# AIoT-MLSys-Lab/Mercury

Measured on AMD Instinct MI355X. Metric: images/sec (whole node) + sampler overhead %, ResNet-18 CIFAR-10 DP 1/2/4/8 GPU, higher is better.
Workload: dtype bf16; 1 GPU; model=resnet18, dataset=cifar10-shape (32x32x3, 10 classes), global_batch=32, per_gpu_batch=32, presample_pool=320, optimizer=adam, parallelism=dp1, sampler=importance (loss + 0.5*EMA), with replacement

## Files before the change

csrc/bindings.cpp:

```cpp
#include <pybind11/pybind11.h>
#include <pybind11/stl.h>

#include <stdexcept>
#include <string>
#include <vector>

#include "kernels.h"

int igemm_read_stamps(unsigned long long* host, int n);
int conv_bwd_pair_sc_launch(const bf16* dyA, const bf16* wtA, const ConvGeom& gA_in,
                            const EpiParams& eA_in, int bm, int bn, int splits, const bf16* xA,
                            const WgradGeom& wgA_in, float* dwA, int wbm, int wbn, int wsplits,
                            const bf16* dyB, const bf16* wtB, const ConvGeom& gtB,
                            const EpiParams& eB_in, int HB, int WB, int NB, const bf16* xB,
                            const WgradGeom& wgB_in, float* dwB, int wsplitsB, hipStream_t st);
int igemm_dual_launch(const bf16* srcA, const bf16* wtA, const ConvGeom& gA, const EpiParams& eA,
                      int splitsA, const bf16* srcB, const bf16* wtB, const ConvGeom& gB,
                      const EpiParams& eB, int splitsB, int bm, int bn, hipStream_t st);
int hconv_read_stamps(unsigned long long* host, int n);
void hconv_configure(int grid, int waves, int wm8);
std::string comm_unique_id();
uintptr_t comm_init(const std::string& id_bytes, int rank, int nranks);
void comm_destroy(uintptr_t c);
void comm_allreduce(uintptr_t c, uintptr_t buf, long long count, int dtype, int avg, uintptr_t st);
void comm_allgather(uintptr_t c, uintptr_t send, uintptr_t recv, long long count, int dtype,
                    uintptr_t st);
void comm_broadcast(uintptr_t c, uintptr_t buf, long long count, int dtype, int root, uintptr_t st);
void comm_ring_allreduce(uintptr_t c, uintptr_t buf, long long count, uintptr_t work, int avg,
                         uintptr_t st);
void add_f32(float* dst, const float* src, long long n, hipStream_t s);
void xgmi_pack(const float* src, void* xbuf, long long n, int bf, hipStream_t st);
void xgmi_reduce_scatter(const void* const* peers, int W, int rank, long long n, int bf,
                         float scale, hipStream_t st);
void xgmi_all_gather(const void* const* peers, int W, long long n, int bf, float* dst,
                     hipStream_t st);
int xgmi_max_ranks();
void xgmi_barrier(const void* const* flag_areas, int W, int rank, unsigned* epoch,
                  double timeout_s, int* err, hipStream_t st);
int xgmi_flag_bytes();
std::string xgmi_ipc_handle(uintptr_t ptr);
uintptr_t xgmi_ipc_open(const std::string& handle);
uintptr_t xgmi_malloc(long long bytes);
// ... 57 lines not shown
                       int bn, int H, int W, int N, uintptr_t st, uintptr_t bw_out, uintptr_t bw_y,
                       uintptr_t bw_stats, uintptr_t bw_y2, uintptr_t bw_stats2, uintptr_t bw_sums,
                       float bw_inv_count, float bw_eps, int bw_act) {
    ConvGeom g{SH, SW, SC, H, W, R, Sk, stride, pad, R * Sk * SC / 8, Ncols, N * H * W};
    EpiParams e{P<bf16>(dx), ldo, nullptr, nullptr, 0, N * H * W, accumulate, nullptr,
                P<const bf16>(bw_out), P<const bf16>(bw_y), P<const float>(bw_stats),
                P<const bf16>(bw_y2), P<const float>(bw_stats2), P<float>(bw_sums), bw_inv_count,
                bw_eps, bw_act};
    const int ok = dgrad_s2_launch(P<const bf16>(dy), P<const bf16>(wt), g, e, bm, bn, H, W, N,
                                   S(st));
    if (ok) check_launch("dgrad_s2");
    return ok;
  });
  m.def("conv_bwd_pair_s2", [](uintptr_t dy, uintptr_t wt, uintptr_t dx, int ldo, int accumulate,
                               int SH, int SW, int SC, int R, int Sk, int stride, int pad,
                               int Ncols, int bm, int bn, int H, int W, int N, uintptr_t bw_out,
                               uintptr_t bw_y, uintptr_t bw_stats, uintptr_t bw_y2,
                               uintptr_t bw_stats2, uintptr_t bw_sums, float bw_inv_count,
                               float bw_eps, int bw_act, uintptr_t x, uintptr_t dw, int C, int Pp,
                               int Q, int K, int Creal, int wbm, int wbn, int wsplits,
                               uintptr_t wslab, uintptr_t st) {
    ConvGeom g{SH, SW, SC, H, W, R, Sk, stride, pad, R * Sk * SC / 8, Ncols, N * H * W};
    EpiParams e{P<bf16>(dx), ldo, nullptr, nullptr, 0, N * H * W, accumulate, nullptr,
                P<const bf16>(bw_out), P<const bf16>(bw_y), P<const float>(bw_stats),
                P<const bf16>(bw_y2), P<const float>(bw_stats2), P<float>(bw_sums), bw_inv_count,
                bw_eps, bw_act};
    WgradGeom wg{N, H, W, C, Pp, Q, K, R, Sk, stride, pad, Creal, nullptr, P<float>(wslab)};
    const int ok = conv_bwd_pair_s2_launch(P<const bf16>(dy), P<const bf16>(wt), g, e, bm, bn, H,
                                           W, N, P<const bf16>(x), wg, P<float>(dw), wbm, wbn,
                                           wsplits, S(st));
    if (ok) check_launch("conv_bwd_pair_s2");
    return ok;
  });
  m.attr("SUMS_R") = SUMS_R;
  m.def("pgemm", [](uintptr_t a, uintptr_t b, uintptr_t out, uintptr_t stats, int M, int N, int K,
                    int ldo, int stats_ld, int group_rows, long long a_bytes, long long b_bytes,
                    long long out_bytes, int H, int W, int Pp, int Q, int stride, int bn, int grid,
                    uintptr_t st, int p_mode, uintptr_t p_stats, uintptr_t p_rmean,
                    uintptr_t p_rvar, uintptr_t p_gamma, uintptr_t p_beta, float p_inv_count,
                    float p_eps, int p_act, int p_group_rows, int p_G, uintptr_t p_coef,
                    uintptr_t p_res, uintptr_t p_keep, long long p_res_bytes,
                    long long p_keep_bytes, long long p_coef_bytes) {
    const long long lim = 0xFFFFFF00LL;
    if (a_bytes >= lim || b_bytes >= lim || out_bytes >= lim || p_res_bytes >= lim ||
        p_keep_bytes >= lim || p_coef_bytes >= lim)
      throw std::invalid_argument("pgemm: tensors must be < 4 GB (32-bit buffer offsets)");
    PgemmArgs g{P<const bf16>(a), P<const bf16>(b), P<bf16>(out), P<float>(stats), M, N, K, ldo,
                stats_ld, group_rows, (unsigned)a_bytes, (unsigned)b_bytes, (unsigned)out_bytes,
                H, W, Pp, Q, stride};
    PgemmPro pr{p_mode, P<const float>(p_stats), P<const float>(p_rmean), P<const float>(p_rvar),
                P<const float>(p_gamma), P<const float>(p_beta), p_inv_count, p_eps, p_act,
                p_group_rows, p_G, P<float>(p_coef), P<const bf16>(p_res), P<bf16>(p_keep),
                (unsigned)p_res_bytes, (unsigned)p_keep_bytes, (unsigned)p_coef_bytes};
    const int ok = bn == 0 ? pwconv_launch(g, S(st), &pr) : pgemm_launch(g, bn, grid, S(st), &pr);
    check_launch(bn == 0 ? "pwconv" : "pgemm");
    return ok;
  });
  m.def("igemm_pro", [](uintptr_t src, uintptr_t wt, uintptr_t out, int ldo, uintptr_t bias,
                        uintptr_t stats, int stats_ld, int group_rows, uintptr_t slab, int SH,
                        int SW, int SC, int RP, int RQ, int R, int Sk, int stride, int pad, int Kc,
                        int Ncols, int M, int bm, int bn, int splits, uintptr_t st,
                        uintptr_t p_stats, uintptr_t p_rmean, uintptr_t p_rvar, uintptr_t p_gamma,
                        uintptr_t p_beta, uintptr_t p_keep, int p_group_rows, float p_inv_count,
                        float p_eps, int p_act, int p_keep_tap, uintptr_t p_res) {
    ConvGeom g{SH, SW, SC, RP, RQ, R, Sk, stride, pad, Kc, Ncols, M};
    EpiParams e{P<bf16>(out), ldo, P<const float>(bias), P<float>(stats), stats_ld, group_rows, 0,
// ... 595 lines not shown
```

csrc/igemm.hip:

```cpp

#include <stdexcept>
#include <string>

#include "conv_epi.h"
#include "wgrad_body.h"

namespace {


__device__ __attribute__((aligned(16))) bf16 g_zero_page[64];

MA_DEV int swz(int row, int chunk) { return chunk ^ (row & 7); }

template <int BM, int BN>
constexpr int nt_occ() { return BM * BN >= 256 * 128 ? 1 : 2; }


template <bool TRANS>
MA_DEV void row_init(const ConvGeom& g, int m, int& off, int& h, int& w) {
  const int pq = g.RP * g.RQ;
  const int mm = m < g.M ? m : 0;
  const int n = udiv24(mm, pq, 1.f / (float)pq), rem = mm - n * pq;
  const int p = udiv24(rem, g.RQ, 1.f / (float)g.RQ), q = rem - p * g.RQ;
  off = m < g.M ? n * g.SH * g.SW : -1;
// ... 336 lines not shown
    unsigned long long lap[4] = {0, 0, 0, 0};
    unsigned long long tl = __builtin_amdgcn_s_memtime();
#endif
    int buf = 0;
    for (int kt = kt0; kt < kt1; ++kt) {
      const bool more = kt + 1 < kt1;
      if (more) load_stage(kt + 1, ra, rb);
      MA_LAP(0, tl);
      const bf16* a = sA + buf * Smem<BM, BN>::STAGE;
      mma_stage<BM, BN>(a, a + BM * BK, acc, lane, wm, wn);
      MA_LAP(1, tl);
      if (more) store_stage(buf ^ 1, ra, rb);
      MA_LAP(2, tl);
      __syncthreads();
      MA_LAP(3, tl);
      buf ^= 1;
    }
#ifdef MERCURY_STAMPS
    if (threadIdx.x == 0) {
      const int b_ = blockIdx.x + blockIdx.y * gridDim.x;
      if (b_ < 8192)
        for (int q = 0; q < 4; ++q) g_stamps[b_][4 + q] = lap[q];
    }
#endif
  } else if constexpr (EARLY) {
    pf.init(e, g.M, g.Ncols, m0, n0);
    if (pf_tail) epi_prefetch(pf, e, m0, n0, g.Ncols);
  }
  MA_STAMP(2);
  finish<BM, BN, 2, BWT, EARLY>(acc, smem, e, g.M, g.Ncols, m0, n0, bx, by, gx, gy, &pf);
  MA_STAMP(3);
}


template <int BM, int BN>
constexpr int PAIR_PF() { return BM * BN <= 64 * 128 ? 2 : 1; }

template <int BM, int BN, bool TRANS, int PF = 1>
__global__ __launch_bounds__(NT, (nt_occ<BM, BN>())) void igemm_nt_kernel(const bf16* __restrict__ src,
                                                          const bf16* __restrict__ wt,
                                                          ConvGeom g, EpiParams e,
                                                          int ktiles_per_split) {
  __shared__ __attribute__((aligned(16))) char smem[Smem<BM, BN>::bytes(2)];
  const ProParams none{};
  const int bx = gridDim.y == 1 ? xcd_tile(blockIdx.x, gridDim.x) : blockIdx.x;
  igemm_nt_body<BM, BN, TRANS, false, PF>(src, wt, g, e, ktiles_per_split, smem, bx, blockIdx.y,
                                          gridDim.x, gridDim.y, none);
}

template <int BM, int BN>
__global__ __launch_bounds__(NT, (nt_occ<BM, BN>())) void igemm_pro_kernel(const bf16* __restrict__ src,
                                                           const bf16* __restrict__ wt,
                                                           ConvGeom g, EpiParams e,
                                                           int ktiles_per_split, ProParams pro) {
  __shared__ __attribute__((aligned(16))) char smem[Smem<BM, BN>::bytes(2)];
  const int bx = gridDim.y == 1 ? xcd_tile(blockIdx.x, gridDim.x) : blockIdx.x;
  igemm_nt_body<BM, BN, false, true>(src, wt, g, e, ktiles_per_split, smem, bx,
                                     blockIdx.y, gridDim.x, gridDim.y, pro);
}

template <int BM, int BN, bool TRANS>
void launch_main(const bf16* src, const bf16* wt, const ConvGeom& g, const EpiParams& e, int per,
                 dim3 grid, hipStream_t st) {
  if constexpr (PAIR_PF<BM, BN>() == 2) {
#ifndef MERCURY_FWD_PF1
    if (grid.x * grid.y <= 512) {
      hipLaunchKernelGGL((igemm_nt_kernel<BM, BN, TRANS, 2>), grid, dim3(NT), 0, st, src, wt, g, e,
                         per);
      return;
    }
#endif
  }
  hipLaunchKernelGGL((igemm_nt_kernel<BM, BN, TRANS>), grid, dim3(NT), 0, st, src, wt, g, e, per);
}

inline void ig_grid(const ConvGeom& g, int BM, int BN, int splits, int& gx, int& per, int& gy) {
  const int mtiles = (g.M + BM - 1) / BM, ntiles = (g.Ncols + BN - 1) / BN;
  const int ktiles = (g.Kc + 7) / 8;
  splits = splits < 1 ? 1 : (splits > ktiles ? ktiles : splits);
  per = (ktiles + splits - 1) / splits;
  gy = (ktiles + per - 1) / per;
  gx = mtiles * ntiles;
  if (gx > SEM_INTS) gy = 1, per = ktiles;
}

template <int BM, int BN, bool TRANS>
void launch_cfg(const bf16* src, const bf16* wt, const ConvGeom& g, EpiParams e, int splits,
                hipStream_t st, const ProParams* pro) {
  int gx, per, gy;
  ig_grid(g, BM, BN, splits, gx, per, gy);
  if (gy == 1) e.slab = nullptr;
  if (pro != nullptr && !TRANS) {
    hipLaunchKernelGGL((igemm_pro_kernel<BM, BN>), dim3(gx, gy), dim3(NT), 0, st, src, wt, g, e,
                       per, *pro);
    return;
  }
  launch_main<BM, BN, TRANS>(src, wt, g, e, per, dim3(gx, gy), st);
}

struct IgProb {
  const bf16* src;
  const bf16* wt;
  ConvGeom g;
  EpiParams e;
  int per, gx, gy;
};

template <int BM, int BN, int PF>
__global__ __launch_bounds__(NT, (nt_occ<BM, BN>())) void igemm_dual_kernel(IgProb A, IgProb B) {
  __shared__ __attribute__((aligned(16))) char smem[Smem<BM, BN>::bytes(2)];
  const ProParams none{};
  int b = blockIdx.x;
  const bool first = b < A.gx * A.gy;
  if (!first) b -= A.gx * A.gy;
  const IgProb& p = first ? A : B;
  const int bx0 = b % p.gx, by = b / p.gx;
  const int bx = p.gy == 1 ? xcd_tile(bx0, p.gx) : bx0;
  igemm_nt_body<BM, BN, false, false, PF>(p.src, p.wt, p.g, p.e, p.per, smem, bx, by, p.gx, p.gy,
                                          none);
}

template <int BM, int BN>
// ... 30 lines not shown
  const int c = (b >= sg.pre[1]) + (b >= sg.pre[2]) + (b >= sg.pre[3]);
  EpiParams ec = e;
  ec.rm_hc = sg.hc[c];
  ec.rm_wc = sg.wc[c];
  ec.rm_h = sg.H;
  ec.rm_w = sg.W;
  ec.rm_ph = c >> 1;
  ec.rm_pw = c & 1;
  const ProParams none{};
  const int bx = b - sg.pre[c];
  igemm_nt_body<BM, BN, false, false, PF, true>(dy, wt, sg.g[c], ec, 1 << 20, smem, bx, 0,
                                                sg.pre[c + 1] - sg.pre[c], 1, none);
}

template <int BM, int BN>
void s2_cfg(const bf16* dy, const bf16* wt, const S2Geom& sg, const EpiParams& e, hipStream_t st) {
  const int grid = sg.pre[4];
  if (grid == 0) return;
  if constexpr (PAIR_PF<BM, BN>() == 2) {
    if (grid <= 512) {
      hipLaunchKernelGGL((dgrad_s2_kernel<BM, BN, 2>), dim3(grid), dim3(NT), 0, st, dy, wt, sg, e);
      return;
    }
  }
  hipLaunchKernelGGL((dgrad_s2_kernel<BM, BN, 1>), dim3(grid), dim3(NT), 0, st, dy, wt, sg, e);
}

template <int DBM, int DBN, int WBM, int WBN>
__global__ __launch_bounds__(NT, 2) void bwd_pair_kernel(const bf16* __restrict__ dy,
                                                          const bf16* __restrict__ wt, ConvGeom g,
                                                          EpiParams e, int dper, int dgx, int dgy,
                                                          const bf16* __restrict__ x,
                                                          WgradGeom wg, float* __restrict__ dw,
                                                          int wper, int wgx, int wgy) {
  constexpr int DB = Smem<DBM, DBN>::bytes(2), WB = wgb::WgSmem<WBM, WBN>::BYTES;
  __shared__ __attribute__((aligned(16))) char smem[DB > WB ? DB : WB];
  const int nw = wgx * wgy;
  const int b = blockIdx.x;
  if (b < nw) {
    wgb::wgrad_body<WBM, WBN>(dy, x, wg, dw, wper, (bf16*)smem, b % wgx, b / wgx, wgy);
  } else {
    const int d = b - nw;
    const ProParams none{};
    igemm_nt_body<DBM, DBN, true, false, PAIR_PF<DBM, DBN>()>(dy, wt, g, e, dper, smem, d % dgx,
                                                               d / dgx, dgx, dgy, none);
  }
}

template <int DBM, int DBN, int WBM, int WBN>
__global__ __launch_bounds__(NT, 2) void bwd_pair_s2_kernel(const bf16* __restrict__ dy,
                                                             const bf16* __restrict__ wt,
                                                             S2Geom sg, EpiParams e,
                                                             const bf16* __restrict__ x,
                                                             WgradGeom wg, float* __restrict__ dw,
                                                             int wper, int wgx, int wgy) {
  constexpr int DB = Smem<DBM, DBN>::bytes(2), WB = wgb::WgSmem<WBM, WBN>::BYTES;
  __shared__ __attribute__((aligned(16))) char smem[DB > WB ? DB : WB];
  const int nw = wgx * wgy;
  const int b = blockIdx.x;
  if (b < nw) {
    wgb::wgrad_body<WBM, WBN>(dy, x, wg, dw, wper, (bf16*)smem, b % wgx, b / wgx, wgy);
    return;
  }
  const int d = b - nw;
  const int c = (d >= sg.pre[1]) + (d >= sg.pre[2]) + (d >= sg.pre[3]);
  EpiParams ec = e;
  ec.rm_hc = sg.hc[c];
  ec.rm_wc = sg.wc[c];
  ec.rm_h = sg.H;
  ec.rm_w = sg.W;
  ec.rm_ph = c >> 1;
  ec.rm_pw = c & 1;
  const ProParams none{};
  igemm_nt_body<DBM, DBN, false, false, PAIR_PF<DBM, DBN>(), true>(
      dy, wt, sg.g[c], ec, 1 << 20, smem, d - sg.pre[c], 0, sg.pre[c + 1] - sg.pre[c], 1, none);
}

struct PairProb {
  const bf16* dy;
  const bf16* wt;
  ConvGeom g;
  EpiParams e;
  int dper, dgx, dgy;
  const bf16* x;
  WgradGeom wg;
  float* dw;
  int wper, wgx, wgy;
};
struct S2PairProb {
  const bf16* dy;
  const bf16* wt;
  S2Geom sg;
  EpiParams e;
  const bf16* x;
  WgradGeom wg;
  float* dw;
  int wper, wgx, wgy;
};

template <int DBM, int DBN, int WBM, int WBN>
__global__ __launch_bounds__(NT, 2) void bwd_pair_sc_kernel(PairProb A, S2PairProb B) {
  constexpr int DB = Smem<DBM, DBN>::bytes(2), WB = wgb::WgSmem<WBM, WBN>::BYTES;
  constexpr int SB = Smem<64, 64>::bytes(2), SWB = wgb::WgSmem<64, 64>::BYTES;
  constexpr int M1 = DB > WB ? DB : WB, M2 = SB > SWB ? SB : SWB;
  __shared__ __attribute__((aligned(16))) char smem[M1 > M2 ? M1 : M2];
  const ProParams none{};
  int b = blockIdx.x;
  const int nwA = A.wgx * A.wgy, nA = nwA + A.dgx * A.dgy;
  if (b < nA) {
    if (b < nwA) {
      wgb::wgrad_body<WBM, WBN>(A.dy, A.x, A.wg, A.dw, A.wper, (bf16*)smem, b % A.wgx, b / A.wgx,
                                A.wgy);
    } else {
      const int d = b - nwA;
      igemm_nt_body<DBM, DBN, true, false, PAIR_PF<DBM, DBN>()>(A.dy, A.wt, A.g, A.e, A.dper, smem,
                                                                 d % A.dgx, d / A.dgx, A.dgx,
                                                                 A.dgy, none);
    }
    return;
  }
  b -= nA;
  const int nwB = B.wgx * B.wgy;
  if (b < nwB) {
    wgb::wgrad_body<64, 64>(B.dy, B.x, B.wg, B.dw, B.wper, (bf16*)smem, b % B.wgx, b / B.wgx, B.wgy);
    return;
  }
  const int d = b - nwB;
  const int c = (d >= B.sg.pre[1]) + (d >= B.sg.pre[2]) + (d >= B.sg.pre[3]);
  EpiParams ec = B.e;
  ec.rm_hc = B.sg.hc[c];
  ec.rm_wc = B.sg.wc[c];
  ec.rm_h = B.sg.H;
  ec.rm_w = B.sg.W;
  ec.rm_ph = c >> 1;
  ec.rm_pw = c & 1;
  igemm_nt_body<64, 64, false, false, PAIR_PF<64, 64>(), true>(
      B.dy, B.wt, B.sg.g[c], ec, 1 << 20, smem, d - B.sg.pre[c], 0, B.sg.pre[c + 1] - B.sg.pre[c],
      1, none);
}

template <int DBM, int DBN, int WBM, int WBN>
void pair_cfg(const bf16* dy, const bf16* wt, const ConvGeom& g, EpiParams e, int splits,
              const bf16* x, WgradGeom wg, float* dw, int wsplits, hipStream_t st) {
  int dgx, dper, dgy, wgx, wper, wgy;
  ig_grid(g, DBM, DBN, splits, dgx, dper, dgy);
  if (dgy == 1) e.slab = nullptr;
  wgb::wg_grid(wg, WBM, WBN, wsplits, wgx, wper, wgy);
  if (wgx > wgb::WG_SEM_INTS) wg.slab = nullptr;
  hipLaunchKernelGGL((bwd_pair_kernel<DBM, DBN, WBM, WBN>), dim3(dgx * dgy + wgx * wgy), dim3(NT),
                     0, st, dy, wt, g, e, dper, dgx, dgy, x, wg, dw, wper, wgx, wgy);
}

}

int igemm_read_stamps(unsigned long long* host, int n) {
#ifdef MERCURY_STAMPS
  return hipMemcpyFromSymbol(host, HIP_SYMBOL(g_stamps), sizeof(unsigned long long) * 12 * n) ==
         hipSuccess;
#else
  (void)host;
  (void)n;
  return 0;
#endif
}


size_t igemm_slab_bytes(const ConvGeom& g, int bm, int bn, int splits) {
  const size_t mtiles = (g.M + bm - 1) / bm, ntiles = (g.Ncols + bn - 1) / bn;
  return SEM_INTS * 4 + (size_t)splits * mtiles * ntiles * bm * bn * 4;
}

const bf16* conv_zero_page();
static const bf16* zero_page() { return conv_zero_page(); }

const bf16* conv_zero_page() {
  static const bf16* zp = nullptr;
  if (!zp) {
    void* p = nullptr;
    (void)hipGetSymbolAddress(&p, HIP_SYMBOL(g_zero_page));
    zp = (const bf16*)p;
  }
  return zp;
}

void igemm_ranges(ConvGeom& g, long long images, const char* who) {
// ... 147 lines not shown
    wgb::wg_grid(wg, WBM_, WBN_, wsplits, wgx, wper, wgy);                                 \
    if (wgx > wgb::WG_SEM_INTS) wg.slab = nullptr;                                         \
    hipLaunchKernelGGL((bwd_pair_s2_kernel<DBM_, DBN_, WBM_, WBN_>),                        \
                       dim3(sg.pre[4] + wgx * wgy), dim3(NT), 0, st, dy, wt, sg, e, x, wg, dw, \
                       wper, wgx, wgy);                                                    \
    return 1;                                                                              \
  }
  MA_W(64, 64, 64, 64)
  MA_W(64, 64, 128, 128)
  MA_W(64, 64, 64, 128)
  MA_W(64, 64, 128, 64)
#undef MA_W
  return 0;
}

int conv_bwd_pair_sc_launch(const bf16* dyA, const bf16* wtA, const ConvGeom& gA_in,
                            const EpiParams& eA_in, int bm, int bn, int splits, const bf16* xA,
                            const WgradGeom& wgA_in, float* dwA, int wbm, int wbn,
                            int wsplits, const bf16* dyB, const bf16* wtB, const ConvGeom& gtB,
                            const EpiParams& eB_in, int HB, int WB, int NB, const bf16* xB,
                            const WgradGeom& wgB_in, float* dwB, int wsplitsB,
                            hipStream_t st) {
  PairProb A;
  A.dy = dyA;
  A.wt = wtA;
  A.g = gA_in;
  A.g.zero = zero_page();
  igemm_ranges(A.g, geom_images(A.g), "conv_bwd_pair_sc");
  A.e = eA_in;
  A.x = xA;
  A.wg = wgA_in;
  A.wg.zero = A.g.zero;
  A.dw = dwA;
  ig_grid(A.g, bm, bn, splits, A.dgx, A.dper, A.dgy);
  if (A.dgy == 1) A.e.slab = nullptr;
  wgb::wg_grid(A.wg, wbm, wbn, wsplits, A.wgx, A.wper, A.wgy);
  if (A.wgx > wgb::WG_SEM_INTS) A.wg.slab = nullptr;
  S2PairProb B;
  if (!s2_geom(gtB, 64, 64, HB, WB, NB, eB_in.ldo, B.sg)) return 0;
  B.dy = dyB;
  B.wt = wtB;
  B.e = eB_in;
  B.e.slab = nullptr;
  B.x = xB;
  B.wg = wgB_in;
  B.wg.zero = A.g.zero;
  B.dw = dwB;
  wgb::wg_grid(B.wg, 64, 64, wsplitsB, B.wgx, B.wper, B.wgy);
  if (B.wgx > wgb::WG_SEM_INTS) B.wg.slab = nullptr;
  if (A.wg.slab != nullptr && A.wg.slab == B.wg.slab) return 0;
  const int grid = A.wgx * A.wgy + A.dgx * A.dgy + B.wgx * B.wgy + B.sg.pre[4];
#define MA_SC(DBM_, DBN_, WBM_, WBN_)                                                       \
  if (bm == DBM_ && bn == DBN_ && wbm == WBM_ && wbn == WBN_) {                             \
    hipLaunchKernelGGL((bwd_pair_sc_kernel<DBM_, DBN_, WBM_, WBN_>), dim3(grid), dim3(NT), 0, st, \
                       A, B);                                                                \
    return 1;                                                                                \
  }
  MA_SC(64, 64, 64, 64)
  MA_SC(64, 64, 128, 128)
#undef MA_SC
  return 0;
}

int conv_bwd_pair_launch(const bf16* dy, const bf16* wt, const ConvGeom& g_in, const EpiParams& e,
                         int bm, int bn, int splits, const bf16* x, const WgradGeom& wg_in,
                         float* dw, int wbm, int wbn, int wsplits, hipStream_t st) {
  ConvGeom g = g_in;
// ... 26 lines not shown
```

mercury_amd/config.py:

```python
from __future__ import annotations

import argparse
import dataclasses
import time
from dataclasses import dataclass


@dataclass
class Config:
    alpha: float = 0.5
    ema_alpha: float = 0.9
    presample_batches: int = 10
    importance: bool = True
    global_ema: bool = False
    exchange_scores: bool = False
    score: str = 'loss'
    sampler: str = 'alias'
    dataset: str = 'cifar10'
    data_dir: str = './data/cifar10'
    num_classes: int = 10
    noniid: bool = True
    partition: str = 'hetero'
    dirichlet_alpha: float = 0.5
    batch_size: int = 32
# ... 61 lines not shown
        p = cls.add_args(argparse.ArgumentParser('mercury_amd'))
        ns, _ = p.parse_known_args(argv)
        return cls(**{f.name: getattr(ns, f.name) for f in dataclasses.fields(cls)})

    def to_dict(self):
        return dataclasses.asdict(self)


@dataclass
class EngineOptions:
    hconv: str = '1'
    hconv_persist: bool = True
    hconv_persist_grid: int = 0
    hconv_persist_waves: int = 8
    hconv_persist_wm8: int = 4
    hconv_swa: bool = True
    hconv_pad: bool = True
    pro_plans: bool = True
    hconv_row: str = 'score'
    hconv_plans: str = ''
    pgemm: bool = True
    pwconv: bool = True
    pwconv_plain: bool = True
    stem: bool = True
    dual_fwd: bool = True
    role_prio: str = 'auto'
    dual_bwd: bool = True
    fuse_bn_fwd: bool = True
    res_pro: bool = True
    dw_pro: bool = True
    dw_pair: bool = True
    head_bw: bool = True
    dgrad_s2: bool = True
    fused_opt: bool = True
    comm_events: bool = True
    rccl_one_rank: bool = False
    head_bn: bool = True
    bucket_calib: str = 'auto'
    last_bucket_mb: float = 1.0
    score_min_blocks: int = 128
    debug_log: bool = False
    persist_bn: str = 'row'

    @classmethod
    def from_env(cls, base=None):
        import os
        import re
        o = dataclasses.replace(base) if base is not None else cls()
        spec = os.environ.get('MERCURY_ENGINE_OPTS', '').strip()
        if not spec:
            return o
        types = {f.name: f.type for f in dataclasses.fields(cls)}
        for item in re.split(r',(?=[a-z_][a-z0-9_]*=)', spec):
            if '=' not in item:
                raise ValueError('MERCURY_ENGINE_OPTS: %r is not name=value' % item)
            k, v = item.split('=', 1)
            k = k.strip()
            if k not in types:
                raise ValueError('MERCURY_ENGINE_OPTS: unknown option %r (EngineOptions)' % k)
            t = types[k]
            if t in ('bool', bool):
                val = v.strip().lower() in ('1', 'true', 'yes', 'on')
            elif t in ('int', int):
                val = int(v)
            elif t in ('float', float):
                val = float(v)
# ... 6 lines not shown
```

mercury_amd/engine/schedule.py:

```python
from __future__ import annotations

from collections import namedtuple

from ..ops import conv, hconv, tune
from ..ops.conv import (ConvSpec, cpad8, dgrad_plan, fwd_plan, pgemm_ok, pgemm_plain_wins,
                        pgemm_plan, pgemm_pro_wins, pro_ok, pro_plan, pwconv_ok,
                        pwconv_plain_wins, pwconv_pro_wins, slab_bytes, stem_ok, wgrad_plan)

ACTS = ('relu', 'relu6', 'none')


class ModePlan(object):

    def __init__(self, N, group_imgs, train):
        self.N = N
        self.group_imgs = group_imgs
        self.train = train
        self.G = 1 if not group_imgs else N // group_imgs
        self.spec = {}
        self.plan = {}
        self.slab = 0
        self.coef = 0
        self.stats = {}
        self.nstats = 0
        self.pool = {}
        self.hw = {}
        self.final_hw = 0
        self.final_C = 0


def apply_globals(opts):
    hconv.configure(opts)
    conv.DGRAD_S2 = opts.dgrad_s2


def plan_mode(lw, opts, N, H, W, group_imgs, train):
    apply_globals(opts)
    mp = ModePlan(N, group_imgs, train)
    persist_bn = opts.persist_bn if opts.persist_bn in ('0', '1', 'row', 'stat') else (
        '1' if str(opts.persist_bn).lower() in ('true', 'on', 'yes') else '0')
    C = cpad8(lw.in_channels)
    for bi, blk in enumerate(lw.blocks):
        h, w = H, W
        main_hw = None
        for u in blk.units + ([blk.shortcut] if blk.shortcut else []):
            if u is blk.shortcut:
                main_hw = (h, w)
                h, w = H, W
            sp = ConvSpec(N, h, w, u.C, u.K, u.R, u.R, u.stride, u.pad)
            if group_imgs:
                sp.group_rows = group_imgs * sp.P * sp.Q
            mp.spec[u.name] = sp
            if not u.depthwise:
                mb = opts.score_min_blocks if group_imgs else 0
                mp.plan[u.name, 'fwd'] = p = tune.fwd_plan_for(
                    sp, fwd_plan(sp, min_blocks=mb) if mb else fwd_plan(sp))
                slab = slab_bytes(sp.M, sp.K, *p[:3])
                pp = pro_plan(sp) if opts.pro_plans else None
                if pp is not None:
                    mp.plan[u.name, 'fwd_pro'] = pp
                    slab = max(slab, slab_bytes(sp.M, sp.K, *pp))
                if opts.pgemm and pgemm_ok(sp) and u.b_seg is None:
                    mp.plan[u.name, 'pgemm'] = pgemm_plan(sp)
                    mp.coef = max(mp.coef, mp.G * 2 * sp.Cp)
                if opts.stem and stem_ok(sp) and bi == 0 and u is blk.units[0]:
                    mp.plan[u.name, 'stem'] = True
# ... 289 lines not shown
```

mercury_amd/ops/conv.py:

```python
from __future__ import annotations

import math
from dataclasses import dataclass

import torch

from . import _chk, lib, ptr, stream_ptr

CU = 256
WG_SEM_INTS = 1024


def cpad8(c):
    return (c + 7) // 8 * 8


@dataclass
class ConvSpec:
    N: int
    H: int
    W: int
    C: int
    K: int
    R: int
# ... 379 lines not shown
_NO_BW = (0, 0, 0, 0, 0, 0, 0.0, 0.0, 0)
_ACT = {None: 0, 'none': 0, 'relu': 1, 'relu6': 2}


def _bw_args(bw, Mx, Cp):
    if bw is None:
        return _NO_BW
    for k in ('out', 'y', 'y2'):
        if bw.get(k) is not None:
            _chk(bw[k], torch.bfloat16, 'bw.' + k, Mx * Cp)
    _chk(bw['sums'], torch.float32, 'bw.sums', int(getattr(lib(), 'SUMS_R', 1)) * 3 * Cp)
    _chk(bw['stats'], torch.float32, 'bw.stats', 2 * Cp)
    return (ptr(bw['out']), ptr(bw['y']), ptr(bw['stats']), ptr(bw.get('y2')),
            ptr(bw.get('stats2')), ptr(bw['sums']), 1.0 / Mx, float(bw.get('eps', 1e-5)),
            _ACT[bw.get('act')])


DGRAD_S2 = True


def dgrad_s2_ok(spec: ConvSpec):
    return (DGRAD_S2 and spec.stride == 2 and spec.R == spec.S and spec.K % 64 == 0 and
            ((spec.R == 3 and spec.pad == 1) or (spec.R == 1 and spec.pad == 0)))


def dgrad_s2_plan(spec: ConvSpec):
    M = spec.N * spec.H * spec.W
    N = spec.Cp
    bn = 128 if N >= 128 else 64
    bm = 128 if math.ceil(M / 128) * math.ceil(N / bn) >= 2 * CU else 64
    return bm, bn, 1


def conv_dgrad(dy, wt, dx, spec: ConvSpec, slab=None, plan=None, accumulate=False, bw=None):
    if spec.stride not in (1, 2):
        raise ValueError('dgrad supports stride 1/2')
    if spec.K % 8:
        raise ValueError('dgrad needs K % 8 == 0')
    Cp = spec.Cp
    _chk(dy, torch.bfloat16, 'dy', spec.M * spec.K)
    _chk(wt, torch.bfloat16, 'wt', Cp * spec.R * spec.S * spec.K)
    _chk(dx, torch.bfloat16, 'dx', spec.N * spec.H * spec.W * Cp)
    Mx = spec.N * spec.H * spec.W
    if dgrad_s2_ok(spec):
        bm, bn, _ = plan or dgrad_s2_plan(spec)
        if lib().dgrad_s2(ptr(dy), ptr(wt), ptr(dx), Cp, int(accumulate), spec.P, spec.Q,
                          spec.K, spec.R, spec.S, spec.stride, spec.pad, Cp, bm, bn, spec.H,
                          spec.W, spec.N, stream_ptr(), *_bw_args(bw, Mx, Cp)):
            return dx
    bm, bn, splits = plan or dgrad_plan(spec)
    if splits > 1:
        slab = _slab(slab, slab_bytes(Mx, Cp, bm, bn, splits), dy.device)
    lib().igemm(ptr(dy), ptr(wt), ptr(dx), Cp, 0, 0, Cp, Mx, int(accumulate),
                ptr(slab) if splits > 1 else 0,
                spec.P, spec.Q, spec.K, spec.H, spec.W, spec.R, spec.S, spec.stride, spec.pad,
                spec.R * spec.S * spec.K // 8, Cp, Mx, bm, bn, splits, True, stream_ptr(),
                *_bw_args(bw, Mx, Cp))
    return dx


def wgrad_slab_bytes(spec: ConvSpec, plan):
    bm, bn, splits = plan[:3]
    ncols = spec.R * spec.S * spec.Cp
    gx = math.ceil(spec.K / bm) * math.ceil(ncols / bn)
    ptiles = math.ceil(spec.M / 64)
    splits = max(1, min(splits, ptiles))
    per = math.ceil(ptiles / splits)
    gy = math.ceil(ptiles / per)
    if gy <= 1 or gx > WG_SEM_INTS:
        return 0
    return WG_SEM_INTS * 4 + gx * gy * bm * bn * 4


def conv_wgrad(dy, x, dw, spec: ConvSpec, plan=None, slab=None):
    _chk(dy, torch.bfloat16, 'dy', spec.M * spec.K)
    _chk(x, torch.bfloat16, 'x', spec.N * spec.H * spec.W * spec.Cp)
    _chk(dw, torch.float32, 'dw', spec.K * spec.R * spec.S * spec.C)
    if spec.K % 8:
        raise ValueError('wgrad needs K % 8 == 0')
    _wg_range(spec)
    bm, bn, splits = (plan or wgrad_plan(spec))[:3]
    lib().wgrad(ptr(dy), ptr(x), ptr(dw), spec.N, spec.H, spec.W, spec.Cp, spec.P, spec.Q,
                spec.K, spec.R, spec.S, spec.stride, spec.pad, spec.C, bm, bn, splits,
                _wslab_ptr(spec, (bm, bn, splits), slab), stream_ptr())
    return dw
# ... 10 lines not shown
        return 0
    if slab.numel() * slab.element_size() < need:
        raise ValueError('wgrad slab too small (%d < %d bytes)'
                         % (slab.numel() * slab.element_size(), need))
    return ptr(slab)


def conv_bwd(dy, wt, dx, x, dw, spec: ConvSpec, dplan=None, wplan=None, slab=None,
             accumulate=False, bw=None, wslab=None):
    if spec.stride not in (1, 2) or spec.K % 8:
        raise ValueError('conv_bwd needs stride 1/2 and K % 8 == 0')
    Cp = spec.Cp
    _chk(dy, torch.bfloat16, 'dy', spec.M * spec.K)
    _chk(wt, torch.bfloat16, 'wt', Cp * spec.R * spec.S * spec.K)
    _chk(dx, torch.bfloat16, 'dx', spec.N * spec.H * spec.W * Cp)
    _chk(x, torch.bfloat16, 'x', spec.N * spec.H * spec.W * Cp)
    _chk(dw, torch.float32, 'dw', spec.K * spec.R * spec.S * spec.C)
    _wg_range(spec)
    bm, bn, splits = dplan or dgrad_plan(spec)
    wbm, wbn, wsplits = (wplan or wgrad_plan(spec))[:3]
    Mx = spec.N * spec.H * spec.W
    if dgrad_s2_ok(spec):
        if spec.N <= 32 and lib().conv_bwd_pair_s2(
                ptr(dy), ptr(wt), ptr(dx), Cp, int(accumulate), spec.P, spec.Q, spec.K, spec.R,
                spec.S, spec.stride, spec.pad, Cp, 64, 64, spec.H, spec.W, spec.N,
                *_bw_args(bw, Mx, Cp), ptr(x), ptr(dw), Cp, spec.P, spec.Q, spec.K, spec.C, wbm,
                wbn, wsplits, _wslab_ptr(spec, (wbm, wbn, wsplits), wslab), stream_ptr()):
            return dx, dw
        conv_wgrad(dy, x, dw, spec, plan=(wbm, wbn, wsplits), slab=wslab)
        conv_dgrad(dy, wt, dx, spec, plan=dgrad_s2_plan(spec), accumulate=accumulate, bw=bw)
        return dx, dw
    if splits > 1:
        slab = _slab(slab, slab_bytes(Mx, Cp, bm, bn, splits), dy.device)
    ok = lib().conv_bwd_pair(
        ptr(dy), ptr(wt), ptr(dx), Cp, int(accumulate), ptr(slab) if splits > 1 else 0,
        spec.P, spec.Q, spec.K, spec.H, spec.W, spec.R, spec.S, spec.stride, spec.pad,
        spec.R * spec.S * spec.K // 8, Cp, Mx, bm, bn, splits, *_bw_args(bw, Mx, Cp),
        ptr(x), ptr(dw), spec.N, spec.H, spec.W, Cp, spec.P, spec.Q, spec.K, spec.C, wbm, wbn,
        wsplits, _wslab_ptr(spec, (wbm, wbn, wsplits), wslab), stream_ptr())
    if not ok:
        conv_wgrad(dy, x, dw, spec, plan=(wbm, wbn, wsplits), slab=wslab)
        conv_dgrad(dy, wt, dx, spec, slab=slab, plan=(bm, bn, splits), accumulate=accumulate,
                   bw=bw)
    return dx, dw


def conv_bwd_sc(a, b):
    sa, sb = a['spec'], b['spec']
    if sa.stride != 1 or sa.K % 8 or not dgrad_s2_ok(sb) or sb.N > 32:
        return False
    bm, bn, splits = a.get('dplan') or dgrad_plan(sa)
    wbm, wbn, wsplits = (a.get('wplan') or wgrad_plan(sa))[:3]
    sbm, sbn, ssplits = (b.get('wplan') or wgrad_plan(sb))[:3]
    if (sbm, sbn) != (64, 64):
        return False
    for d, sp in ((a, sa), (b, sb)):
        _chk(d['dy'], torch.bfloat16, 'dy', sp.M * sp.K)
        _chk(d['wt'], torch.bfloat16, 'wt', sp.Cp * sp.R * sp.S * sp.K)
        _chk(d['dx'], torch.bfloat16, 'dx', sp.N * sp.H * sp.W * sp.Cp)
        _chk(d['x'], torch.bfloat16, 'x', sp.N * sp.H * sp.W * sp.Cp)
        _chk(d['dw'], torch.float32, 'dw', sp.K * sp.R * sp.S * sp.C)
        _wg_range(sp)
    Mx = sa.N * sa.H * sa.W
    slab = a.get('slab')
    if splits > 1:
        slab = _slab(slab, slab_bytes(Mx, sa.Cp, bm, bn, splits), a['dy'].device)
    ta = (ptr(a['dy']), ptr(a['wt']), ptr(a['dx']), sa.Cp, int(a.get('accumulate', False)),
          ptr(slab) if splits > 1 else 0, sa.P, sa.Q, sa.K, sa.H, sa.W, sa.R, sa.S, sa.stride,
          sa.pad, sa.R * sa.S * sa.K // 8, sa.Cp, Mx, bm, bn, splits,
          *_bw_args(a.get('bw'), Mx, sa.Cp), ptr(a['x']), ptr(a['dw']), sa.N, sa.H, sa.W, sa.Cp,
          sa.P, sa.Q, sa.K, sa.C, wbm, wbn, wsplits, 0)
    Mb = sb.N * sb.H * sb.W
    tb = (ptr(b['dy']), ptr(b['wt']), ptr(b['dx']), sb.Cp, int(b.get('accumulate', False)),
          sb.P, sb.Q, sb.K, sb.R, sb.S, sb.stride, sb.pad, sb.Cp, 64, 64, sb.H, sb.W, sb.N,
          *_bw_args(None, Mb, sb.Cp), ptr(b['x']), ptr(b['dw']), sb.Cp, sb.P, sb.Q, sb.K, sb.C,
          sbm, sbn, ssplits, 0)
    return bool(lib().conv_bwd_pair_sc(ta, tb, stream_ptr()))


def to_nhwc(x, cpad=None):
    n, c, h, w = x.shape
    cp = cpad or cpad8(c)
    out = torch.zeros(n, h, w, cp, dtype=torch.bfloat16, device=x.device)
    out[..., :c] = x.permute(0, 2, 3, 1).to(torch.bfloat16)
    return out


def from_nhwc(y, c=None):
    c = c or y.shape[-1]
    return y[..., :c].permute(0, 3, 1, 2).float()


def pack_conv_weight(w_kcrs):
    k, c, r, s = w_kcrs.shape
    krsc = torch.zeros(k, r, s, cpad8(c), dtype=torch.bfloat16, device=w_kcrs.device)
    krsc[..., :c] = w_kcrs.permute(0, 2, 3, 1).to(torch.bfloat16)
    crsk = w_kcrs.permute(1, 2, 3, 0).contiguous().to(torch.bfloat16)
    return krsc.contiguous(), crsk
```

Measured before the change: 27040 trained images/s.

## Add halo-tiled stride-1 3x3 dgrad kernel reusing dy tile across taps

Adds a specialized dgrad body for stride-1 3x3 pad-1 convolutions with 64x64 tiles. It loads a padded halo of dy pixels into LDS once per 64-channel chunk and reuses it for all nine filter taps, streaming only the weight slices per tap. This avoids the implicit-GEMM path reloading overlapping dy rows nine times. The path is wired into the standalone, pair and shortcut-pair launches behind a config flag. In exchange it adds more syncthreads per chunk, since each tap only double-buffers weights in the last chunk, and brings extra eligibility checks.

```diff
diff --git a/csrc/bindings.cpp b/csrc/bindings.cpp
--- a/csrc/bindings.cpp
+++ b/csrc/bindings.cpp
@@ -8,6 +8,8 @@
 #include "kernels.h"
 
 int igemm_read_stamps(unsigned long long* host, int n);
+void igemm_set_dgrad_halo(int on);
+int igemm_dgrad_halo_ok(const ConvGeom& g, int bm, int bn, int splits);
 int conv_bwd_pair_sc_launch(const bf16* dyA, const bf16* wtA, const ConvGeom& gA_in,
                             const EpiParams& eA_in, int bm, int bn, int splits, const bf16* xA,
                             const WgradGeom& wgA_in, float* dwA, int wbm, int wbn, int wsplits,
@@ -131,6 +133,13 @@
     if (ok) check_launch("conv_bwd_pair_s2");
     return ok;
   });
+  m.def("set_dgrad_halo", [](int on) { igemm_set_dgrad_halo(on); });
+  m.def("dgrad_halo_ok", [](int N, int H, int W, int K, int R, int Sk, int stride, int pad, int Cp,
+                            int bm, int bn, int splits) {
+    const int Pp = (H + 2 * pad - R) / stride + 1, Q = (W + 2 * pad - Sk) / stride + 1;
+    ConvGeom g{Pp, Q, K, H, W, R, Sk, stride, pad, R * Sk * K / 8, Cp, N * H * W};
+    return igemm_dgrad_halo_ok(g, bm, bn, splits);
+  });
   m.attr("SUMS_R") = SUMS_R;
   m.def("pgemm", [](uintptr_t a, uintptr_t b, uintptr_t out, uintptr_t stats, int M, int N, int K,
                     int ldo, int stats_ld, int group_rows, long long a_bytes, long long b_bytes,
diff --git a/csrc/igemm.hip b/csrc/igemm.hip
--- a/csrc/igemm.hip
+++ b/csrc/igemm.hip
@@ -392,6 +392,183 @@
   MA_STAMP(3);
 }
 
+constexpr int HALO_PIX = 192;
+constexpr int HALO_LD = HALO_PIX / 32;
+constexpr int HALO_BYTES = HALO_PIX * BK * 2 + 2 * 64 * BK * 2;
+
+MA_DEV void dgrad_halo_body(const bf16* __restrict__ dy, const bf16* __restrict__ wt,
+                            const ConvGeom& g, const EpiParams& e, int chunks_per_split,
+                            char* smem, int bx, int by, int gx, int gy) {
+  constexpr int BM = 64, BN = 64, TM = 2, TN = 2, BR = 2;
+  bf16* sH = (bf16*)smem;
+  bf16* sB = sH + HALO_PIX * BK;
+
+  const int tid = threadIdx.x, lane = tid & 63, w = tid >> 6;
+  const int wm = w >> 1, wn = w & 1;
+  const int ntn = (g.Ncols + BN - 1) / BN;
+  const int mt = bx / ntn, nt = bx - mt * ntn;
+  const int m0 = mt * BM, n0 = nt * BN;
+  MA_STAMP(0);
+  const int K = g.SC, nchunks = (K + 63) >> 6;
+  const int c0 = by * chunks_per_split;
+  const int c1 = min(nchunks, c0 + chunks_per_split);
+  const int cc = tid & 7;
+  const auto rsa = __builtin_amdgcn_make_buffer_rsrc((void*)dy, 0, g.a_bytes, IG_RSRC_FLAGS);
+  const auto rsb = __builtin_amdgcn_make_buffer_rsrc((void*)wt, 0, g.b_bytes, IG_RSRC_FLAGS);
+
+  const int H = g.RP, W = g.RQ, hw = H * W;
+  const int lw = __builtin_ctz(W);
+  const bool whole = hw <= 64;
+  const int PR = whole ? H : 64 >> lw;
+  const int lpp = __builtin_ctz(PR) + lw;
+  const int pitch = W + 2, PRH = PR + 2;
+  const int swa = W == 4 ? 4 : 0;
+  const int hpix = (64 >> lpp) * PRH * pitch;
+  const int img0 = whole ? m0 >> lpp : m0 / hw;
+  const int row0 = whole ? 0 : (m0 - img0 * hw) >> lw;
+
+  unsigned hsrc[HALO_LD];
+  int hdst[HALO_LD];
+  {
+    const float rp = 1.f / (float)pitch, rr = 1.f / (float)PRH;
+#pragma unroll
+    for (int i = 0; i < HALO_LD; ++i) {
+      const int j = (tid >> 3) + 32 * i;
+      const int hrg = udiv24(j, pitch, rp), hc = j - hrg * pitch;
+      const int piece = udiv24(hrg, PRH, rr), hr = hrg - piece * PRH;
+      const int sr = row0 + hr - 1, sc = hc - 1;
+      const bool ok = j < hpix && (unsigned)sr < (unsigned)H && (unsigned)sc < (unsigned)W;
+      hsrc[i] = ok ? (unsigned)((img0 + piece) * hw + sr * W + sc) * (unsigned)K * 2u : IG_OOB;
+      hdst[i] = j * BK + ((cc ^ ((hc + swa * hrg) & 7)) << 3);
+    }
+  }
+  unsigned boff[BR];
+  bool bval[BR];
+#pragma unroll
+  for (int i = 0; i < BR; ++i) {
+    const int n = n0 + (tid >> 3) + 32 * i;
+    bval[i] = n < g.Ncols;
+    boff[i] = (unsigned)n * (unsigned)(g.Kc * 8) * 2u;
+  }
+  int fpix[TM], fkey[TM];
+#pragma unroll
+  for (int tm = 0; tm < TM; ++tm) {
+    const int i = wm * (BM / 2) + tm * 16 + (lane & 15);
+    const int piece = i >> lpp, lr = (i >> lw) & (PR - 1), lc = i & (W - 1);
+    const int hrg = piece * PRH + lr + 2, hc = lc + 2;
+    fpix[tm] = hrg * pitch + hc;
+    fkey[tm] = hc + swa * hrg;
+  }
+
+  auto load_halo = [&](int ci, u32x4 (&rh)[HALO_LD]) {
+    const int ch = ci * 64 + cc * 8;
+    const bool chv = ch < K;
+#pragma unroll
+    for (int i = 0; i < HALO_LD; ++i)
+      rh[i] = ig_load16(rsa, chv && hsrc[i] != IG_OOB ? hsrc[i] + (unsigned)ch * 2u : IG_OOB);
+  };
+  auto store_halo = [&](const u32x4 (&rh)[HALO_LD]) {
+#pragma unroll
+    for (int i = 0; i < HALO_LD; ++i) *(u32x4*)(sH + hdst[i]) = rh[i];
+  };
+  auto load_w = [&](int tap, int ci, u32x4 (&rb)[BR]) {
+    const int ch = ci * 64 + cc * 8;
+    const bool kval = tap < 9 && ch < K;
+    const unsigned bcol = (unsigned)(tap * K + ch) * 2u;
+#pragma unroll
+    for (int i = 0; i < BR; ++i) rb[i] = ig_load16(rsb, kval && bval[i] ? boff[i] + bcol : IG_OOB);
+  };
+  auto store_w = [&](int buf, const u32x4 (&rb)[BR]) {
+    bf16* b = sB + buf * BN * BK;
+#pragma unroll
+    for (int i = 0; i < BR; ++i) {
+      const int row = (tid >> 3) + 32 * i;
+      *(u32x4*)(b + row * BK + swz(row, cc) * 8) = rb[i];
+    }
+  };
+
+  f32x4 acc[TM][TN];
+#pragma unroll
+  for (int i = 0; i < TM; ++i)
+#pragma unroll
+    for (int j = 0; j < TN; ++j) acc[i][j] = f32x4{0.f, 0.f, 0.f, 0.f};
+
+  auto mma_tap = [&](int tap, const bf16* b) {
+    const int r = (tap * 11) >> 5, s = tap - 3 * r;
+    const int d = r * pitch + s, kd = s + swa * r;
+#pragma unroll
+    for (int kk = 0; kk < 2; ++kk) {
+      const int chunk = kk * 4 + (lane >> 4);
+      bf16x8 fa[TM], fb[TN];
+#pragma unroll
+      for (int tm = 0; tm < TM; ++tm) {
+        const int key = (fkey[tm] - kd) & 7;
+        fa[tm] = *(const bf16x8*)(sH + (fpix[tm] - d) * BK + ((chunk ^ key) << 3));
+      }
+#pragma unroll
+      for (int tn = 0; tn < TN; ++tn) {
+        const int row = wn * (BN / 2) + tn * 16 + (lane & 15);
+        fb[tn] = *(const bf16x8*)(b + row * BK + swz(row, chunk) * 8);
+      }
+#pragma unroll
+      for (int tm = 0; tm < TM; ++tm)
+#pragma unroll
+        for (int tn = 0; tn < TN; ++tn)
+          acc[tm][tn] = __builtin_amdgcn_mfma_f32_16x16x32_bf16(fb[tn], fa[tm], acc[tm][tn], 0, 0, 0);
+    }
+  };
+
+  EpiPf<BM, BN, true> pf;
+  const bool pf_tail = EPI_PF_ALL || e.slab == nullptr;
+
+#pragma nounroll
+  for (int ci = c0; ci + 1 < c1; ++ci) {
+    u32x4 rh[HALO_LD], rb[BR];
+    load_halo(ci, rh);
+    store_halo(rh);
+#pragma nounroll
+    for (int tap = 0; tap < 9; ++tap) {
+      load_w(tap, ci, rb);
+      store_w(0, rb);
+      __syncthreads();
+      mma_tap(tap, sB);
+      __syncthreads();
+    }
+  }
+  if (c0 < c1) {
+    const int ci = c1 - 1;
+    u32x4 rh[HALO_LD], rb0[BR], rb1[BR];
+    load_halo(ci, rh);
+    load_w(0, ci, rb0);
+    load_w(1, ci, rb1);
+    pf.init(e, g.M, g.Ncols, m0, n0);
+    store_halo(rh);
+    store_w(0, rb0);
+    __syncthreads();
+    int kt = 0;
+#pragma nounroll
+    for (; kt + 2 < 9; kt += 2) {
+      load_w(kt + 2, ci, rb0);
+      mma_tap(kt, sB);
+      store_w(1, rb1);
+      __syncthreads();
+      load_w(kt + 3, ci, rb1);
+      mma_tap(kt + 1, sB + BN * BK);
+      store_w(0, rb0);
+      __syncthreads();
+    }
+    if (pf_tail) epi_prefetch(pf, e, m0, n0, g.Ncols);
+    mma_tap(kt, sB);
+    __syncthreads();
+  } else {
+    pf.init(e, g.M, g.Ncols, m0, n0);
+    if (pf_tail) epi_prefetch(pf, e, m0, n0, g.Ncols);
+  }
+  MA_STAMP(2);
+  finish<BM, BN, 2, true, true>(acc, smem, e, g.M, g.Ncols, m0, n0, bx, by, gx, gy, &pf);
+  MA_STAMP(3);
+}
+
 
 template <int BM, int BN>
 constexpr int PAIR_PF() { return BM * BN <= 64 * 128 ? 2 : 1; }
@@ -419,6 +596,45 @@
                                      blockIdx.y, gridDim.x, gridDim.y, pro);
 }
 
+__global__ __launch_bounds__(NT, 2) void dgrad_halo_kernel(const bf16* __restrict__ dy,
+                                                           const bf16* __restrict__ wt, ConvGeom g,
+                                                           EpiParams e, int chunks_per_split) {
+  __shared__ __attribute__((aligned(16))) char smem[HALO_BYTES];
+  const int bx = gridDim.y == 1 ? xcd_tile(blockIdx.x, gridDim.x) : blockIdx.x;
+  dgrad_halo_body(dy, wt, g, e, chunks_per_split, smem, bx, blockIdx.y, gridDim.x, gridDim.y);
+}
+
+int g_dgrad_halo = 1;
+
+bool dgrad_halo_ok(const ConvGeom& g, int bm, int bn, int splits) {
+  if (!g_dgrad_halo || bm != 64 || bn != 64) return false;
+  if (g.R != 3 || g.S != 3 || g.stride != 1 || g.pad != 1) return false;
+  const int H = g.RP, W = g.RQ, K = g.SC;
+  if (H <= 0 || W <= 0 || g.SH != H || g.SW != W) return false;
+  if (g.trb >= 0 || g.ldb != 0 || K % 8 || g.Kc != 9 * (K / 8)) return false;
+  if (g.M % 64 || g.M % (H * W)) return false;
+  int pieces, rows;
+  if (64 % (H * W) == 0) {
+    pieces = 64 / (H * W);
+    rows = H;
+  } else if (64 % W == 0 && H % (64 / W) == 0) {
+    pieces = 1;
+    rows = 64 / W;
+  } else {
+    return false;
+  }
+  if (pieces * (rows + 2) * (W + 2) > HALO_PIX) return false;
+  return ((K + 63) / 64) % (splits < 1 ? 1 : splits) == 0;
+}
+
+inline void halo_grid(const ConvGeom& g, int splits, int& gx, int& per, int& gy) {
+  const int nchunks = (g.SC + 63) / 64;
+  gy = splits < 1 ? 1 : splits;
+  gx = (g.M / 64) * ((g.Ncols + 63) / 64);
+  if (gx > SEM_INTS) gy = 1;
+  per = nchunks / gy;
+}
+
 template <int BM, int BN, bool TRANS>
 void launch_main(const bf16* src, const bf16* wt, const ConvGeom& g, const EpiParams& e, int per,
                  dim3 grid, hipStream_t st) {
@@ -448,6 +664,16 @@
 void launch_cfg(const bf16* src, const bf16* wt, const ConvGeom& g, EpiParams e, int splits,
                 hipStream_t st, const ProParams* pro) {
   int gx, per, gy;
+  if constexpr (TRANS && BM == 64 && BN == 64) {
+    if (dgrad_halo_ok(g, BM, BN, splits)) {
+      halo_grid(g, splits, gx, per, gy);
+      if (gx * gy <= 512) {
+        if (gy == 1) e.slab = nullptr;
+        hipLaunchKernelGGL(dgrad_halo_kernel, dim3(gx, gy), dim3(NT), 0, st, src, wt, g, e, per);
+        return;
+      }
+    }
+  }
   ig_grid(g, BM, BN, splits, gx, per, gy);
   if (gy == 1) e.slab = nullptr;
   if (pro != nullptr && !TRANS) {
@@ -544,15 +770,24 @@
                                                           EpiParams e, int dper, int dgx, int dgy,
                                                           const bf16* __restrict__ x,
                                                           WgradGeom wg, float* __restrict__ dw,
-                                                          int wper, int wgx, int wgy) {
+                                                          int wper, int wgx, int wgy, int halo) {
   constexpr int DB = Smem<DBM, DBN>::bytes(2), WB = wgb::WgSmem<WBM, WBN>::BYTES;
+  static_assert(DBM * DBN != 64 * 64 || WB >= HALO_BYTES, "the halo fits the wgrad's LDS");
   __shared__ __attribute__((aligned(16))) char smem[DB > WB ? DB : WB];
   const int nw = wgx * wgy;
   const int b = blockIdx.x;
   if (b < nw) {
+    MA_STAMP(0);
     wgb::wgrad_body<WBM, WBN>(dy, x, wg, dw, wper, (bf16*)smem, b % wgx, b / wgx, wgy);
+    MA_STAMP(3);
   } else {
     const int d = b - nw;
+    if constexpr (DBM == 64 && DBN == 64) {
+      if (halo) {
+        dgrad_halo_body(dy, wt, g, e, dper, smem, d % dgx, d / dgx, dgx, dgy);
+        return;
+      }
+    }
     const ProParams none{};
     igemm_nt_body<DBM, DBN, true, false, PAIR_PF<DBM, DBN>()>(dy, wt, g, e, dper, smem, d % dgx,
                                                                d / dgx, dgx, dgy, none);
@@ -594,6 +829,7 @@
   ConvGeom g;
   EpiParams e;
   int dper, dgx, dgy;
+  int halo;
   const bf16* x;
   WgradGeom wg;
   float* dw;
@@ -615,6 +851,7 @@
   constexpr int DB = Smem<DBM, DBN>::bytes(2), WB = wgb::WgSmem<WBM, WBN>::BYTES;
   constexpr int SB = Smem<64, 64>::bytes(2), SWB = wgb::WgSmem<64, 64>::BYTES;
   constexpr int M1 = DB > WB ? DB : WB, M2 = SB > SWB ? SB : SWB;
+  static_assert(SWB >= HALO_BYTES, "the halo fits the shortcut wgrad's LDS");
   __shared__ __attribute__((aligned(16))) char smem[M1 > M2 ? M1 : M2];
   const ProParams none{};
   int b = blockIdx.x;
@@ -625,6 +862,12 @@
                                 A.wgy);
     } else {
       const int d = b - nwA;
+      if constexpr (DBM == 64 && DBN == 64) {
+        if (A.halo) {
+          dgrad_halo_body(A.dy, A.wt, A.g, A.e, A.dper, smem, d % A.dgx, d / A.dgx, A.dgx, A.dgy);
+          return;
+        }
+      }
       igemm_nt_body<DBM, DBN, true, false, PAIR_PF<DBM, DBN>()>(A.dy, A.wt, A.g, A.e, A.dper, smem,
                                                                  d % A.dgx, d / A.dgx, A.dgx,
                                                                  A.dgy, none);
@@ -655,14 +898,22 @@
 void pair_cfg(const bf16* dy, const bf16* wt, const ConvGeom& g, EpiParams e, int splits,
               const bf16* x, WgradGeom wg, float* dw, int wsplits, hipStream_t st) {
   int dgx, dper, dgy, wgx, wper, wgy;
-  ig_grid(g, DBM, DBN, splits, dgx, dper, dgy);
+  const int halo = dgrad_halo_ok(g, DBM, DBN, splits);
+  if (halo) halo_grid(g, splits, dgx, dper, dgy);
+  else ig_grid(g, DBM, DBN, splits, dgx, dper, dgy);
   if (dgy == 1) e.slab = nullptr;
   wgb::wg_grid(wg, WBM, WBN, wsplits, wgx, wper, wgy);
   if (wgx > wgb::WG_SEM_INTS) wg.slab = nullptr;
   hipLaunchKernelGGL((bwd_pair_kernel<DBM, DBN, WBM, WBN>), dim3(dgx * dgy + wgx * wgy), dim3(NT),
-                     0, st, dy, wt, g, e, dper, dgx, dgy, x, wg, dw, wper, wgx, wgy);
-}
-
+                     0, st, dy, wt, g, e, dper, dgx, dgy, x, wg, dw, wper, wgx, wgy, halo);
+}
+
+}
+
+void igemm_set_dgrad_halo(int on) { g_dgrad_halo = on != 0; }
+
+int igemm_dgrad_halo_ok(const ConvGeom& g, int bm, int bn, int splits) {
+  return dgrad_halo_ok(g, bm, bn, splits);
 }
 
 int igemm_read_stamps(unsigned long long* host, int n) {
@@ -876,7 +1127,9 @@
   A.wg = wgA_in;
   A.wg.zero = A.g.zero;
   A.dw = dwA;
-  ig_grid(A.g, bm, bn, splits, A.dgx, A.dper, A.dgy);
+  A.halo = dgrad_halo_ok(A.g, bm, bn, splits);
+  if (A.halo) halo_grid(A.g, splits, A.dgx, A.dper, A.dgy);
+  else ig_grid(A.g, bm, bn, splits, A.dgx, A.dper, A.dgy);
   if (A.dgy == 1) A.e.slab = nullptr;
   wgb::wg_grid(A.wg, wbm, wbn, wsplits, A.wgx, A.wper, A.wgy);
   if (A.wgx > wgb::WG_SEM_INTS) A.wg.slab = nullptr;
diff --git a/mercury_amd/config.py b/mercury_amd/config.py
--- a/mercury_amd/config.py
+++ b/mercury_amd/config.py
@@ -117,6 +117,7 @@
     dw_pair: bool = True
     head_bw: bool = True
     dgrad_s2: bool = True
+    dgrad_halo: bool = True
     fused_opt: bool = True
     comm_events: bool = True
     rccl_one_rank: bool = False
diff --git a/mercury_amd/engine/schedule.py b/mercury_amd/engine/schedule.py
--- a/mercury_amd/engine/schedule.py
+++ b/mercury_amd/engine/schedule.py
@@ -32,6 +32,7 @@
 def apply_globals(opts):
     hconv.configure(opts)
     conv.DGRAD_S2 = opts.dgrad_s2
+    conv.DGRAD_HALO = opts.dgrad_halo
 
 
 def plan_mode(lw, opts, N, H, W, group_imgs, train):
diff --git a/mercury_amd/ops/conv.py b/mercury_amd/ops/conv.py
--- a/mercury_amd/ops/conv.py
+++ b/mercury_amd/ops/conv.py
@@ -435,6 +435,38 @@
     return bm, bn, 1
 
 
+DGRAD_HALO = True
+HALO_PIX = 192
+_halo_sent = None
+
+
+def dgrad_halo_ok(spec: ConvSpec, plan=None):
+    bm, bn, splits = plan or dgrad_plan(spec)
+    if not DGRAD_HALO or (bm, bn) != (64, 64):
+        return False
+    if (spec.R, spec.S, spec.stride, spec.pad) != (3, 3, 1, 1) or spec.K % 8:
+        return False
+    H, W = spec.H, spec.W
+    if (spec.N * H * W) % 64:
+        return False
+    if 64 % (H * W) == 0:
+        pieces, rows = 64 // (H * W), H
+    elif 64 % W == 0 and H % (64 // W) == 0:
+        pieces, rows = 1, 64 // W
+    else:
+        return False
+    if pieces * (rows + 2) * (W + 2) > HALO_PIX:
+        return False
+    return math.ceil(spec.K / 64) % max(1, splits) == 0
+
+
+def _sync_dgrad_halo():
+    global _halo_sent
+    if _halo_sent != DGRAD_HALO:
+        lib().set_dgrad_halo(int(DGRAD_HALO))
+        _halo_sent = DGRAD_HALO
+
+
 def conv_dgrad(dy, wt, dx, spec: ConvSpec, slab=None, plan=None, accumulate=False, bw=None):
     if spec.stride not in (1, 2):
         raise ValueError('dgrad supports stride 1/2')
@@ -454,6 +486,7 @@
     bm, bn, splits = plan or dgrad_plan(spec)
     if splits > 1:
         slab = _slab(slab, slab_bytes(Mx, Cp, bm, bn, splits), dy.device)
+    _sync_dgrad_halo()
     lib().igemm(ptr(dy), ptr(wt), ptr(dx), Cp, 0, 0, Cp, Mx, int(accumulate),
                 ptr(slab) if splits > 1 else 0,
                 spec.P, spec.Q, spec.K, spec.H, spec.W, spec.R, spec.S, spec.stride, spec.pad,
@@ -530,6 +563,7 @@
         return dx, dw
     if splits > 1:
         slab = _slab(slab, slab_bytes(Mx, Cp, bm, bn, splits), dy.device)
+    _sync_dgrad_halo()
     ok = lib().conv_bwd_pair(
         ptr(dy), ptr(wt), ptr(dx), Cp, int(accumulate), ptr(slab) if splits > 1 else 0,
         spec.P, spec.Q, spec.K, spec.H, spec.W, spec.R, spec.S, spec.stride, spec.pad,
@@ -573,6 +607,7 @@
           sb.P, sb.Q, sb.K, sb.R, sb.S, sb.stride, sb.pad, sb.Cp, 64, 64, sb.H, sb.W, sb.N,
           *_bw_args(None, Mb, sb.Cp), ptr(b['x']), ptr(b['dw']), sb.Cp, sb.P, sb.Q, sb.K, sb.C,
           sbm, sbn, ssplits, 0)
+    _sync_dgrad_halo()
     return bool(lib().conv_bwd_pair_sc(ta, tb, stream_ptr()))
 
 
```

Result: no change. 27180 trained images/s, median of 6 (+0.5%).
